# refresh-bio/colord

Measured on AMD Instinct MI355X. Metric: input Gbases/s + archive size vs ref, ONT 50 Gb at 1/2/4/8 MI355X, higher is better.
Workload: dtype u64

## Files before the change

### colord_amd/csrc/anchors.hip

```cpp
#include "common.hpp"
#include "objects.hpp"
#include <algorithm>

struct cl_anchors {
	cl_ctx* ctx = nullptr;
	uint32_t n_reads = 0, c = 0;
	uint64_t n_anchors = 0;
	DevBuf<uint32_t> n_cands;
	DevBuf<uint32_t> cand;
	DevBuf<uint64_t> cand_off;
	DevBuf<uint32_t> anchors;
};

namespace {

struct Arena { const uint64_t* packed; const uint64_t* word_off; const uint32_t* lens; };

__device__ inline uint64_t mmer_at(const Arena& A, uint64_t wb, uint32_t p, uint32_t m)
{
	const uint64_t* w = A.packed + wb + (p >> 5);
	const uint32_t j = p & 31;
	const uint64_t hi = w[0], lo = w[1];
	const uint32_t s = 128 - 2 * (j + m);
	const uint64_t v = (s >= 64) ? (hi >> (s - 64)) : ((hi << (64 - s)) | (lo >> s));
	return v & ((1ULL << (2 * m)) - 1);
}
__device__ inline uint64_t mmer_of(uint64_t hi, uint64_t lo, uint32_t p, uint32_t m)
{
	const uint32_t s = 128 - 2 * ((p & 31) + m);
	const uint64_t v = (s >= 64) ? (hi >> (s - 64)) : ((hi << (64 - s)) | (lo >> s));
	return v & ((1ULL << (2 * m)) - 1);
}
__device__ inline uint64_t revcomp_m(uint64_t x, uint32_t m)
{
	x = ~x; x = __brevll(x);
	x = ((x >> 1) & 0x5555555555555555ULL) | ((x & 0x5555555555555555ULL) << 1);
	return x >> (64 - 2 * m);
}
__device__ inline uint64_t ref_mmer(const Arena& R, uint32_t id, bool rev, uint32_t q, uint32_t m)
{
	const uint32_t len = R.lens[id];
	const uint64_t wb = R.word_off[id];
	return rev ? revcomp_m(mmer_at(R, wb, len - m - q, m), m) : mmer_at(R, wb, q, m);
}

struct BuildSlot { uint64_t key; uint32_t head; uint32_t strands; };
typedef uint2 EncSlot;
constexpr uint32_t LINK_POS = 0x3fffffffu;
__device__ inline uint32_t tag_of(uint64_t hash) { return (uint32_t)((hash * 0xD6E8FEB86659FD93ULL) >> 32); }
__device__ inline uint32_t table_slot(uint64_t hash, uint32_t tsz) { return (uint32_t)(((uint64_t)(uint32_t)(hash >> 17) * tsz) >> 32); }
struct EncTable { EncSlot* slots; const uint64_t* toff; uint32_t* next; const uint64_t* noff; };
constexpr uint32_t REGION_SLOTS = 2048;
constexpr uint64_t KEY_EMPTY = ~0ULL;
constexpr uint32_t NIL = 0xffffffffu;

__global__ void k_table_sizes(const uint32_t* __restrict__ lens, const uint8_t* __restrict__ has_n, const uint32_t* __restrict__ ncand,
                              uint32_t r0, uint32_t r1, uint32_t m, uint32_t x4, uint32_t lds_max_n, uint32_t* __restrict__ tsize, uint32_t* __restrict__ nsize, uint32_t* __restrict__ err)
{
	uint32_t r = r0 + blockIdx.x * blockDim.x + threadIdx.x;
	if (r >= r1) return;
	uint32_t len = lens[r];
	bool active = ncand[r] > 0 && !has_n[r] && len >= m;
	uint32_t n = active ? len - m + 1 : 0;
	if (n <= lds_max_n) n = 0;
	uint32_t t = 0;
	if (n) { t = 16; while (t < 2 * n + n / 2 && t < REGION_SLOTS) t <<= 1; if (t >= REGION_SLOTS) t = (uint32_t)(((uint64_t)n * x4 / 4 + REGION_SLOTS - 1) / REGION_SLOTS * REGION_SLOTS); }
	tsize[r - r0] = t; nsize[r - r0] = n;
}
constexpr uint32_t REGION = REGION_SLOTS, INS_T = 256;
__global__ __launch_bounds__(INS_T) void k_table_insert(Arena A, uint32_t r0, uint32_t r1, uint32_t m, EncTable T, uint32_t* __restrict__ n_distinct,
                                                       uint2* __restrict__ bins , uint32_t* __restrict__ err)
{
	__shared__ BuildSlot reg[REGION];
	__shared__ uint32_t cnt[512], start[513];
	const uint32_t r = r0 + blockIdx.x;
	if (r >= r1) return;
	const uint64_t t0 = T.toff[r - r0]; const uint32_t tsz = (uint32_t)(T.toff[r - r0 + 1] - t0);
	if (!tsz) return;
	const uint64_t n0 = T.noff[r - r0]; const uint32_t n = (uint32_t)(T.noff[r - r0 + 1] - n0);
	const uint64_t wb = A.word_off[r];
	const uint32_t lane = threadIdx.x & 63;
	const uint32_t rs = tsz < REGION ? tsz : REGION, n_reg = tsz / rs, rshift = 31 - (uint32_t)__clz((int)rs);
	uint2* bin = bins + n0;
	uint32_t fresh = 0;
	for (uint32_t rg0 = 0; rg0 < n_reg; rg0 += 512)
	{
		const uint32_t nr = n_reg - rg0 < 512 ? n_reg - rg0 : 512;
		for (uint32_t i = threadIdx.x; i < 512; i += INS_T) cnt[i] = 0;
		__syncthreads();
		for (uint32_t p = threadIdx.x; p < n; p += INS_T)
		{
			const uint64_t xf = mmer_at(A, wb, p, m), xr = revcomp_m(xf, m), x = xf < xr ? xf : xr;
			const uint32_t h = table_slot(hash_mm(x), tsz), rg = (h >> rshift) - rg0;
			if (rg < nr) atomicAdd(&cnt[rg], 1u);
		}
		__syncthreads();
		if (threadIdx.x == 0) { uint32_t a = 0; for (uint32_t i = 0; i < nr; ++i) { start[i] = a; a += cnt[i]; cnt[i] = 0; } start[nr] = a; }
		__syncthreads();
		for (uint32_t p = threadIdx.x; p < n; p += INS_T)
		{
			const uint64_t xf = mmer_at(A, wb, p, m), xr = revcomp_m(xf, m), x = xf < xr ? xf : xr;
			const uint32_t h = table_slot(hash_mm(x), tsz), rg = (h >> rshift) - rg0;
			if (rg < nr) bin[start[rg] + atomicAdd(&cnt[rg], 1u)] = make_uint2(p, h);
		}
		__syncthreads();
		__threadfence_block();
		for (uint32_t rg = 0; rg < nr; ++rg)
		{
			for (uint32_t i = threadIdx.x; i < rs; i += INS_T) { reg[i].key = KEY_EMPTY; reg[i].head = NIL; reg[i].strands = 0; }
			__syncthreads();
			const uint32_t b = start[rg], e = start[rg + 1];
			for (uint32_t i = b + threadIdx.x; i < e; i += INS_T)
			{
				const uint2 ph = bin[i];
				const uint32_t pp = ph.x;
				const uint64_t xf = mmer_at(A, wb, pp, m), xr = revcomp_m(xf, m), x = xf < xr ? xf : xr;
				uint32_t off = ph.y & (rs - 1), tries = 0;
				for (;;)
				{
					unsigned long long old = atomicCAS((unsigned long long*)&reg[off].key, (unsigned long long)KEY_EMPTY, (unsigned long long)x);
					if (old == KEY_EMPTY || old == x) break;
					off = (off + 1) & (rs - 1);
					if (++tries > rs) { atomicOr(err, 2u); break; }
				}
				const uint32_t strand = xf != x ? 1u : 0u;
				T.next[n0 + pp] = atomicExch(&reg[off].head, pp | (strand << 31));
				if (!(atomicOr(&reg[off].strands, 1u << strand) & (1u << strand))) ++fresh;
			}
			__syncthreads();
			EncSlot* dst = T.slots + t0 + (uint64_t)(rg0 + rg) * rs;
			for (uint32_t i = threadIdx.x; i < rs; i += INS_T) dst[i] = make_uint2(reg[i].head == NIL ? 0u : tag_of(hash_mm(reg[i].key)), reg[i].head);
			__syncthreads();
		}
	}
	fresh = wave_sum(fresh);
	if (lane == 0 && fresh) atomicAdd(&n_distinct[r - r0], fresh);
}
struct TaskCfg { uint32_t r0, r1, c, m; uint32_t pe, pr; double frac_always, frac_min, max_mult; };

constexpr uint32_t FILT_WORDS = 2048, STAGE = 128;
__device__ inline uint32_t filt_word(uint64_t hash) { return (uint32_t)(hash >> 46) & (FILT_WORDS - 1); }
__device__ inline uint64_t filt_mask(uint64_t hash) { return (1ull << ((hash >> 40) & 63)) | (1ull << ((hash >> 34) & 63)) | (1ull << ((hash >> 28) & 63)); }
__device__ __host__ inline uint32_t match_segments(uint32_t n, uint32_t seg_n) { return (seg_n == 0 || n <= seg_n + seg_n / 2) ? 1u : (n + seg_n - 1) / seg_n; }
__global__ __launch_bounds__(256) void k_match(Arena A, Arena R, EncTable T, TaskCfg cfg, const uint32_t* __restrict__ cand_refs, const uint32_t* __restrict__ cand_n,
                                              const uint32_t* __restrict__ n_distinct, const uint2* __restrict__ work , uint32_t n_work, uint32_t seg_n,
                                              unsigned long long* __restrict__ n_pairs, uint64_t cap, uint64_t* __restrict__ pairs)
{
	__shared__ unsigned long long filt[FILT_WORDS];
	__shared__ uint64_t stage_all[4][STAGE];
	if (blockIdx.x >= n_work) return;
	const uint32_t rl = work[blockIdx.x].x, seg = work[blockIdx.x].y;
	const uint32_t lane = threadIdx.x & 63, wv = threadIdx.x >> 6;
	const uint32_t r = cfg.r0 + rl;
	const uint64_t t0 = T.toff[rl]; const uint32_t tsz = (uint32_t)(T.toff[rl + 1] - t0);
	const uint32_t n_slots = cand_n[r] < cfg.c ? cand_n[r] : cfg.c;
	if (tsz == 0 || n_slots == 0) return;
	const uint32_t elen = A.lens[r];
	if ((double)n_distinct[rl] < cfg.frac_min * (double)elen && !((double)n_distinct[rl] > cfg.frac_always * (double)elen)) return;
	for (uint32_t i = threadIdx.x; i < FILT_WORDS; i += 256) filt[i] = 0;
	__syncthreads();
	uint32_t p_lo, p_hi;
	{
		const uint64_t ewb = A.word_off[r]; const uint32_t n = elen - cfg.m + 1;
		const uint32_t nseg = match_segments(n, seg_n);
		if (seg >= nseg) return;
		p_lo = (uint32_t)((uint64_t)n * seg / nseg); p_hi = (uint32_t)((uint64_t)n * (seg + 1) / nseg);
		for (uint32_t p = p_lo + threadIdx.x; p < p_hi; p += 256)
		{
			const uint64_t xf = mmer_at(A, ewb, p, cfg.m), xr = revcomp_m(xf, cfg.m);
			const uint64_t hash = hash_mm(xf < xr ? xf : xr);
			atomicOr(&filt[filt_word(hash)], (unsigned long long)filt_mask(hash));
		}
	}
	__syncthreads();
	const uint64_t n0 = T.noff[rl];
	const uint64_t ewb = A.word_off[r];
	uint64_t* stage = stage_all[wv]; uint32_t fill = 0;
	auto flush = [&]() {
		if (!fill) return;
		unsigned long long base = 0;
		if (lane == 0) base = atomicAdd(n_pairs, (unsigned long long)fill);
		base = ((unsigned long long)__shfl((int)(base >> 32), 0, 64) << 32) | (uint32_t)__shfl((int)(uint32_t)base, 0, 64);
		if (base + fill <= cap) for (uint32_t i = lane; i < fill; i += 64) pairs[base + i] = stage[i];
		fill = 0;
	};
	for (uint32_t slot = 0; slot < n_slots; ++slot)
	{
		const uint32_t id = cand_refs[(uint64_t)r * cfg.c + slot], rlen = R.lens[id];
		if (rlen < cfg.m) continue;
		const uint64_t rwb = R.word_off[id];
		const uint32_t nq = rlen - cfg.m + 1, sl = rl * cfg.c + slot;
		const uint32_t PR = cfg.pr; const uint32_t pr_mask = (1u << PR) - 1;
		const uint64_t key_rev = (uint64_t)(2 * sl) << (cfg.pe + PR), key_fwd = (uint64_t)(2 * sl + 1) << (cfg.pe + PR);
		if (threadIdx.x == 0 && seg == 0) atomicAdd(n_pairs + 1, (unsigned long long)nq);
		const uint64_t* rw = R.packed + rwb;
		struct Probe { uint64_t x; uint2 slot; uint32_t h, tag; bool pass, fwd_other, rev_other; };
		auto probe = [&](uint32_t q, uint64_t hi, uint64_t lo) -> Probe
		{
			Probe P{ 0, make_uint2(0u, NIL), 0, 0, false, false, false };
			if (q < nq)
			{
				const uint64_t y = mmer_of(hi, lo, q, cfg.m), z = revcomp_m(y, cfg.m), x = y < z ? y : z;
				const uint64_t hash = hash_mm(x);
				const uint64_t fm = filt_mask(hash);
				if ((filt[filt_word(hash)] & fm) == fm)
				{
					P.pass = true; P.x = x; P.fwd_other = y != x; P.rev_other = z != x;
					P.h = table_slot(hash, tsz); P.tag = tag_of(hash);
					P.slot = T.slots[t0 + P.h];
				}
			}
			return P;
		};
		uint64_t hi1 = 0, lo1 = 0, hi2 = 0, lo2 = 0;
		Probe cur;
		{
			const uint32_t q = wv * 64 + lane;
			uint64_t hi = 0, lo = 0;
			if (q < nq) { hi = rw[q >> 5]; lo = rw[(q >> 5) + 1]; }
			if (q + 256 < nq) { hi1 = rw[(q + 256) >> 5]; lo1 = rw[((q + 256) >> 5) + 1]; }
			cur = probe(q, hi, lo);
		}
		const uint32_t rmask = (tsz < REGION ? tsz : REGION) - 1;
		for (uint32_t q0 = wv * 64; q0 < nq; q0 += 256)
		{
			const uint32_t q = q0 + lane;
			hi2 = 0; lo2 = 0;
			if (q + 512 < nq) { hi2 = rw[(q + 512) >> 5]; lo2 = rw[((q + 512) >> 5) + 1]; }
			const Probe nxt = probe(q + 256, hi1, lo1);
			uint32_t head = NIL, cnt = 0;
			const uint32_t fs = cur.fwd_other ? 1u : 0u, rs_ = cur.rev_other ? 1u : 0u;
			if (cur.pass)
			{
				uint2 sl8 = cur.slot; uint32_t h = cur.h;
				while (sl8.y != NIL)
				{
					if (sl8.x == cur.tag)
					{
						const uint64_t xf = mmer_at(A, ewb, sl8.y & LINK_POS, cfg.m), xr = revcomp_m(xf, cfg.m);
						if ((xf < xr ? xf : xr) == cur.x) { head = sl8.y; break; }
					}
					h = (h & ~rmask) | ((h + 1) & rmask);
					sl8 = T.slots[t0 + h];
				}
				for (uint32_t p = head; p != NIL; p = T.next[n0 + (p & LINK_POS)])
					if ((p & LINK_POS) >= p_lo && (p & LINK_POS) < p_hi) cnt += (uint32_t)((p >> 31) == fs) + (uint32_t)((p >> 31) == rs_);
			}
			cur = nxt; hi1 = hi2; lo1 = lo2;
			if (!__any(cnt != 0)) continue;
			const uint32_t incl = wave_incl_scan(cnt), tot = __shfl(incl, 63, 64);
			const uint64_t kf = key_fwd | (uint64_t)(~q & pr_mask), kr = key_rev | (uint64_t)(~(nq - 1 - q) & pr_mask);
			if (fill + tot > STAGE) flush();
			if (tot <= STAGE)
			{
				uint32_t o = fill + incl - cnt;
				for (uint32_t p = head; p != NIL; p = T.next[n0 + (p & LINK_POS)])
				{
					if ((p & LINK_POS) < p_lo || (p & LINK_POS) >= p_hi) continue;
					const uint64_t pos = (uint64_t)(p & LINK_POS) << PR;
					if ((p >> 31) == fs) stage[o++] = kf | pos;
					if ((p >> 31) == rs_) stage[o++] = kr | pos;
				}
				fill += tot;
				continue;
			}
			unsigned long long base = 0;
			if (lane == 0) base = atomicAdd(n_pairs, (unsigned long long)tot);
			base = ((unsigned long long)__shfl((int)(base >> 32), 0, 64) << 32) | (uint32_t)__shfl((int)(uint32_t)base, 0, 64);
			if (base + tot > cap) continue;
			uint64_t o = base + incl - cnt;
			for (uint32_t p = head; p != NIL; p = T.next[n0 + (p & LINK_POS)])
			{
				if ((p & LINK_POS) < p_lo || (p & LINK_POS) >= p_hi) continue;
				const uint64_t pos = (uint64_t)(p & LINK_POS) << PR;
				if ((p >> 31) == fs) pairs[o++] = kf | pos;
				if ((p >> 31) == rs_) pairs[o++] = kr | pos;
			}
		}
	}
	flush();
}
template<uint32_t MAXN> struct LdsGeom { static constexpr uint32_t SLOTS = ((MAXN + MAXN / 2) + 17) & ~1u, WORDS = (MAXN + 27 + 31) / 32 + 2; };
__device__ inline uint32_t lds_table_slots(uint32_t n) { const uint32_t s = (n + n / 2 + 1) & ~1u; return s < 16 ? 16 : s; }
template<uint32_t MAXN, uint32_t FW, uint32_t NT, uint32_t WAVES_PER_SIMD>
__global__ __launch_bounds__(NT, WAVES_PER_SIMD) void k_match_lds(Arena A, Arena R, TaskCfg cfg, uint32_t min_n, const uint8_t* __restrict__ has_n,
                                                 const uint32_t* __restrict__ cand_refs, const uint32_t* __restrict__ cand_n, uint32_t* __restrict__ n_distinct, uint32_t n_reads,
                                                 unsigned long long* __restrict__ n_pairs, uint64_t cap, uint64_t* __restrict__ pairs, uint32_t dbg)
{
	static_assert(MAXN <= 65535 && (FW & (FW - 1)) == 0 && NT % 64 == 0, "positions are 16-bit links; 0xffff is the empty slot");
	constexpr uint32_t NW = NT / 64, LSTAGE = 64;
	__shared__ unsigned long long filt[FW];
	__shared__ uint64_t rd[LdsGeom<MAXN>::WORDS];
	__shared__ uint32_t slots32[LdsGeom<MAXN>::SLOTS / 2];
	__shared__ uint64_t stage_all[NW][LSTAGE];
	__shared__ uint32_t s_distinct;
	const uint32_t rl = blockIdx.x;
	if (rl >= n_reads) return;
	const uint32_t r = cfg.r0 + rl, m = cfg.m;
	const uint32_t elen = A.lens[r];
	const uint32_t n_slots = cand_n[r] < cfg.c ? cand_n[r] : cfg.c;
	if (n_slots == 0 || has_n[r] || elen < m) return;
	const uint32_t n = elen - m + 1;
	if (n <= min_n || n > MAXN) return;
	const uint32_t lane = threadIdx.x & 63, wv = threadIdx.x >> 6;
	const uint32_t S = lds_table_slots(n);
	const uint16_t* slot16 = (const uint16_t*)slots32;
	{
		const uint64_t* src = A.packed + A.word_off[r];
		const uint32_t nw = (elen + 31) / 32 + 1;
		for (uint32_t i = threadIdx.x; i < nw; i += NT) rd[i] = src[i];
		for (uint32_t i = threadIdx.x; i < FW; i += NT) filt[i] = 0;
		for (uint32_t i = threadIdx.x; i < S / 2; i += NT) slots32[i] = 0xffffffffu;
		if (threadIdx.x == 0) s_distinct = 0;
	}
	__syncthreads();
	if (dbg == 1) return;
	auto own = [&](uint32_t p) -> uint64_t { return mmer_of(rd[p >> 5], rd[(p >> 5) + 1], p, m); };
	auto step = [&](uint32_t off) -> uint32_t { return off + 1 == S ? 0u : off + 1; };
	{
		uint32_t fresh = 0;
		for (uint32_t p = threadIdx.x; p < n; p += NT)
		{
			const uint64_t xf = own(p), xr = revcomp_m(xf, m), hash = hash_mm(xf < xr ? xf : xr);
			atomicOr(&filt[(uint32_t)(hash >> 46) & (FW - 1)], (unsigned long long)filt_mask(hash));
			bool dup = false;
			for (uint32_t off = table_slot(hash, S);;)
			{
				uint32_t* w = &slots32[off >> 1]; const uint32_t sh = (off & 1) * 16;
				const uint32_t old = *(volatile uint32_t*)w, q = (old >> sh) & 0xffffu;
				if (q != 0xffffu) { if (!dup && own(q) == xf) dup = true; off = step(off); continue; }
				if (atomicCAS(w, old, (old & ~(0xffffu << sh)) | (p << sh)) == old) break;
			}
			fresh += dup ? 0u : 1u;
		}
		fresh = wave_sum(fresh);
		if (lane == 0 && fresh) atomicAdd(&s_distinct, fresh);
	}
	__syncthreads();
	const uint32_t nd = s_distinct;
	if (threadIdx.x == 0) n_distinct[rl] = nd;
	if (dbg == 2) return;
	if ((double)nd < cfg.frac_min * (double)elen && !((double)nd > cfg.frac_always * (double)elen)) return;
	uint64_t* stage = stage_all[wv]; uint32_t fill = 0;
	auto flush = [&]() {
		if (!fill) return;
		unsigned long long base = 0;
		if (lane == 0) base = atomicAdd(n_pairs, (unsigned long long)fill);
		base = ((unsigned long long)__shfl((int)(base >> 32), 0, 64) << 32) | (uint32_t)__shfl((int)(uint32_t)base, 0, 64);
		if (base + fill <= cap) for (uint32_t i = lane; i < fill; i += 64) pairs[base + i] = stage[i];
		fill = 0;
	};
	struct Look { uint64_t y, z; uint32_t h0, cnt, nh, hp0, hp1, hf0, hf1; };
	auto look = [&](bool live, uint32_t q, uint64_t hi, uint64_t lo) -> Look {
		Look L{ 0, 0, 0, 0, 0, 0, 0, 0, 0 };
		if (!live) return L;
		L.y = mmer_of(hi, lo, q, m); L.z = revcomp_m(L.y, m);
		const uint64_t hash = hash_mm(L.y < L.z ? L.y : L.z), fm = filt_mask(hash);
		if ((filt[(uint32_t)(hash >> 46) & (FW - 1)] & fm) != fm || dbg == 3) return L;
		L.h0 = table_slot(hash, S);
		for (uint32_t off = L.h0;; off = step(off))
// ... 366 lines not shown
		const uint64_t s = (uint64_t)r * c + i;
		if (i < n)
		{
			const uint32_t t = sel_task[i] & 0x7fffffffu, slot = (t / 2) % c;
			o_cand[4 * s] = cand_refs[(uint64_t)r * c + slot]; o_cand[4 * s + 1] = (t & 1) == 0 ? 1u : 0u;
			o_cand[4 * s + 2] = sel_tot[i]; o_cand[4 * s + 3] = sel_n[i];
			o_task[(uint64_t)rl * c + i] = sel_task[i]; o_count[(uint64_t)rl * c + i] = sel_n[i];
		}
		else { o_cand[4 * s] = ~0u; o_cand[4 * s + 1] = 0; o_cand[4 * s + 2] = 0; o_cand[4 * s + 3] = 0; o_task[(uint64_t)rl * c + i] = ~0u; o_count[(uint64_t)rl * c + i] = 0; }
	}
}
__global__ void k_copy_fix(const uint32_t* __restrict__ o_task, const uint64_t* __restrict__ slot_off, uint64_t n_slots,
                           const uint64_t* __restrict__ pair_off, const uint32_t* __restrict__ anch, uint64_t dst_base, uint32_t* __restrict__ out,
                           TaskCfg cfg, const uint32_t* __restrict__ kanch, const uint64_t* __restrict__ common_off, uint64_t common_base)
{
	const uint64_t s = (uint64_t)blockIdx.x * blockDim.x + threadIdx.x;
	if (s >= n_slots) return;
	const uint32_t tm = o_task[s];
	if (tm == ~0u) return;
	const uint32_t t = tm & 0x7fffffffu;
	const uint32_t n = (uint32_t)(slot_off[s + 1] - slot_off[s]);
	const uint32_t* src = anch + 3 * pair_off[t];
	if (tm & 0x80000000u)
	{
		const uint64_t gs = (uint64_t)cfg.r0 * cfg.c + t / 2;
		const uint64_t o = common_off[gs] - common_base; const uint32_t nk = (uint32_t)(common_off[gs + 1] - common_off[gs]);
		src = kanch + 6 * o + (uint64_t)(t & 1) * 3 * nk;
	}
	uint32_t* dst = out + 3 * (dst_base + slot_off[s]);
	for (uint32_t i = 0; i < 3 * n; ++i) dst[i] = src[i];
	for (uint32_t i = 0; i + 1 < n; ++i)
	{
		const uint32_t end = dst[3 * i + 2] + dst[3 * i];
		if (dst[3 * (i + 1) + 2] < end) { const uint32_t d = end - dst[3 * (i + 1) + 2]; dst[3 * (i + 1) + 2] += d; dst[3 * (i + 1)] -= d; dst[3 * (i + 1) + 1] += d; }
	}
	for (uint32_t i = 0; i + 1 < n; ++i)
	{
		const uint32_t end = dst[3 * i + 1] + dst[3 * i];
		if (dst[3 * (i + 1) + 1] < end) { const uint32_t d = end - dst[3 * (i + 1) + 1]; dst[3 * (i + 1) + 1] += d; dst[3 * (i + 1)] -= d; dst[3 * (i + 1) + 2] += d; }
	}
}
__global__ void k_add_u64(uint64_t* v, uint64_t n, uint64_t c) { uint64_t i = (uint64_t)blockIdx.x * blockDim.x + threadIdx.x; if (i < n) v[i] += c; }
}

extern "C" cl_status cl_anchor_candidates_hifi(cl_ctx* ctx, const cl_reads* reads, const cl_reads* refs, const uint32_t* d_cand_refs, const uint32_t* d_cand_n,
                                               uint32_t c, uint32_t anchor_len, double frac_always, double frac_min, double max_matches_mult,
                                               uint32_t min_anchors, uint32_t kmer_len, uint32_t modulo, const uint64_t* d_common_off, const uint64_t* d_common, cl_anchors** out);
extern "C" cl_status cl_anchor_candidates(cl_ctx* ctx, const cl_reads* reads, const cl_reads* refs, const uint32_t* d_cand_refs, const uint32_t* d_cand_n,
                                          uint32_t c, uint32_t anchor_len, double frac_always, double frac_min, double max_matches_mult,
                                          uint32_t min_anchors, cl_anchors** out)
{
	return cl_anchor_candidates_hifi(ctx, reads, refs, d_cand_refs, d_cand_n, c, anchor_len, frac_always, frac_min, max_matches_mult, min_anchors, 0, 0, nullptr, nullptr, out);
}
extern "C" cl_status cl_anchor_candidates_hifi(cl_ctx* ctx, const cl_reads* reads, const cl_reads* refs, const uint32_t* d_cand_refs, const uint32_t* d_cand_n,
                                               uint32_t c, uint32_t anchor_len, double frac_always, double frac_min, double max_matches_mult,
                                               uint32_t min_anchors, uint32_t kmer_len, uint32_t modulo, const uint64_t* d_common_off, const uint64_t* d_common, cl_anchors** out)
{
	if (!ctx || !reads || !refs || !d_cand_refs || !d_cand_n || !out) return cl_fail(ctx, CL_E_INVALID, "cl_anchor_candidates: null argument");
	const bool hifi = d_common_off != nullptr;
	if (hifi && (kmer_len < 2 || kmer_len > 28 || modulo == 0)) return cl_fail(ctx, CL_E_INVALID, "cl_anchor_candidates_hifi: 2 <= kmer_len <= 28, modulo >= 1");
	if (c == 0 || c > 16 || anchor_len < 2 || anchor_len > 28) return cl_fail(ctx, CL_E_INVALID, "cl_anchor_candidates: 1 <= c <= 16, 2 <= anchor_len <= 28");
	HIP_TRY(ctx, hipSetDevice(ctx->device));
	const uint32_t nr = reads->n_reads, m = anchor_len;
	cl_anchors* X = new cl_anchors(); X->ctx = ctx; X->n_reads = nr; X->c = c;
	std::unique_ptr<cl_anchors> guard(X);
	DEV_ALLOC(ctx, X->n_cands, nr); DEV_ALLOC(ctx, X->cand, (uint64_t)nr * c * 4); DEV_ALLOC(ctx, X->cand_off, (uint64_t)nr * c + 1);
	Arena A{ reads->packed.p, reads->word_off.p, reads->lens.p }, R{ refs->packed.p, refs->word_off.p, refs->lens.p };
	std::vector<uint32_t> h_len(nr);
	if (nr) HIP_TRY(ctx, hipMemcpy(h_len.data(), reads->lens.p, (uint64_t)nr * 4, hipMemcpyDeviceToHost));
	auto bits_for = [](uint64_t v) -> uint32_t { uint32_t b = 1; while ((1ull << b) <= v) ++b; return b; };
	uint32_t max_ref_len = 0;
	if (refs->n_reads)
	{
		std::vector<uint32_t> rl(refs->n_reads);
		HIP_TRY(ctx, hipMemcpy(rl.data(), refs->lens.p, (uint64_t)refs->n_reads * 4, hipMemcpyDeviceToHost));
		for (uint32_t l : rl) max_ref_len = std::max(max_ref_len, l);
	}
	const uint32_t pr_bits = bits_for(max_ref_len);
	const uint64_t BATCH_BASES = 1ull << 28;
	std::vector<DevBuf<uint32_t>> chunks; std::vector<uint64_t> chunk_n;
	uint64_t total_anchors = 0;
	double pairs_per_base = 0.5;
	struct TableBatch {
		uint32_t r0 = 0, r1 = 0, pe = 1; uint64_t acc = 0, nsum = 0;
		DevBuf<uint32_t> n_distinct, next, err; DevBuf<uint64_t> toff, noff; DevBuf<EncSlot> slots; DevBuf<uint2> bins;
		std::vector<uint2> h_work; DevBuf<uint2> work;
		struct SideSync { hipStream_t s = nullptr; ~SideSync() { if (s) (void)hipStreamSynchronize(s); } } sync;
	};
	HIP_TRY(ctx, cl_side_stream(ctx, ctx->side));
	constexpr uint32_t LDS_N_A = 12288, LDS_N_B = 24576, LDS_NT = 1024;
	uint32_t lds_max_n = 0;
	if (const char* e = getenv("COLORD_HIP_ANCHORS_LDS")) lds_max_n = atoi(e) <= 0 ? 0u : (uint32_t)atoi(e) <= LDS_N_A ? LDS_N_A : LDS_N_B;
	const uint32_t match_seg = getenv("COLORD_HIP_MATCH_SEG") ? (uint32_t)std::max(0, atoi(getenv("COLORD_HIP_MATCH_SEG"))) : 16384u;
	const uint32_t lds_dbg = getenv("COLORD_HIP_LDS_DBG") ? (uint32_t)atoi(getenv("COLORD_HIP_LDS_DBG")) : 0u;
	auto prepare = [&](uint32_t r0, std::unique_ptr<TableBatch>& out) -> cl_status {
		out = std::make_unique<TableBatch>();
		TableBatch& B = *out;
		uint32_t r1 = r0; uint64_t acc = 0;
		uint32_t mx = 0;
		while (r1 < nr && (r1 == r0 || acc + h_len[r1] <= BATCH_BASES))
		{
			const uint32_t pe = bits_for(std::max(mx, h_len[r1]));
			if (r1 > r0 && pe + pr_bits + bits_for((r1 - r0 + 1) * 2 * c) > 64) break;
			mx = std::max(mx, h_len[r1]); acc += h_len[r1]; ++r1;
		}
		B.r0 = r0; B.r1 = r1; B.acc = acc; B.pe = bits_for(mx);
		for (uint32_t r = r0; r < r1; ++r)
			for (uint32_t sg = 0, ns = match_segments(h_len[r] >= m ? h_len[r] - m + 1 : 0, match_seg); sg < ns; ++sg) B.h_work.push_back(make_uint2(r - r0, sg));
		if (B.pe + pr_bits + bits_for((r1 - r0) * 2 * c) > 64) return cl_fail(ctx, CL_E_UNSUPPORTED, "cl_anchor_candidates: a read and its candidates are too long for 64-bit match keys");
		const uint32_t nb = r1 - r0;
		const uint32_t table_x4 = 8;
		LaunchOn on(ctx, ctx->side);
		B.sync.s = ctx->side;
		DevBuf<uint32_t> tsize, nsize, err; DEV_ALLOC(ctx, tsize, nb); DEV_ALLOC(ctx, nsize, nb); DEV_ALLOC(ctx, err, 1); DEV_ALLOC(ctx, B.n_distinct, nb);
		HIP_TRY(ctx, hipMemsetAsync(err.p, 0, 4, ctx->side));
		LAUNCH(ctx, k_table_sizes, grid_for(nb, 256), 256, (const uint32_t*)reads->lens.p, (const uint8_t*)reads->has_n.p, d_cand_n, r0, r1, m, table_x4, lds_max_n, tsize.p, nsize.p, err.p);
		DEV_ALLOC(ctx, B.toff, (uint64_t)nb + 1); DEV_ALLOC(ctx, B.noff, (uint64_t)nb + 1);
		uint64_t tsum = 0;
		CL_TRY(dev_exclusive_scan_u64(ctx, tsize.p, B.toff.p, nb, &tsum));
		CL_TRY(dev_exclusive_scan_u64(ctx, nsize.p, B.noff.p, nb, &B.nsum));
		uint32_t herr = 0; HIP_TRY(ctx, hipMemcpyAsync(&herr, err.p, 4, hipMemcpyDeviceToHost, ctx->side)); HIP_TRY(ctx, hipStreamSynchronize(ctx->side));
		DEV_ALLOC(ctx, B.slots, tsum); DEV_ALLOC(ctx, B.next, B.nsum); DEV_ALLOC(ctx, B.bins, B.nsum); DEV_ALLOC(ctx, B.err, 1);
		DEV_ALLOC(ctx, B.work, B.h_work.size() + 1);
		if (!B.h_work.empty()) HIP_TRY(ctx, hipMemcpyAsync(B.work.p, B.h_work.data(), B.h_work.size() * sizeof(uint2), hipMemcpyHostToDevice, ctx->side));
		HIP_TRY(ctx, hipMemsetAsync(B.n_distinct.p, 0, (uint64_t)nb * 4, ctx->side));
		HIP_TRY(ctx, hipMemsetAsync(B.err.p, 0, 4, ctx->side));
		EncTable T{ B.slots.p, B.toff.p, B.next.p, B.noff.p };
		LAUNCHB(ctx, B.nsum * (0.25 + 16.0) , k_table_insert, nb, INS_T, A, r0, r1, m, T, B.n_distinct.p, B.bins.p, B.err.p);
		HIP_TRY(ctx, hipGetLastError());
		return CL_OK;
	};
	std::unique_ptr<TableBatch> cur, nxt;
	if (nr) CL_TRY(prepare(0, cur));
	while (cur)
	{
		const uint32_t r0 = cur->r0, r1 = cur->r1; const uint64_t acc = cur->acc;
		const uint32_t nb = r1 - r0, n_tasks = nb * 2 * c;
		TaskCfg cfg{ r0, r1, c, m, cur->pe, pr_bits, frac_always, frac_min, max_matches_mult };
		HIP_TRY(ctx, hipStreamSynchronize(ctx->stream));
		HIP_TRY(ctx, hipStreamSynchronize(ctx->side));
		cur->sync.s = nullptr;
		{ uint32_t herr = 0; HIP_TRY(ctx, hipMemcpy(&herr, cur->err.p, 4, hipMemcpyDeviceToHost)); if (herr) return cl_fail(ctx, CL_E_UNSUPPORTED, "cl_anchor_candidates: a region of an m-mer table overflowed"); }
		DevBuf<uint32_t>& n_distinct = cur->n_distinct;
		EncTable T{ cur->slots.p, cur->toff.p, cur->next.p, cur->noff.p };
		DevBuf<uint32_t> pair_cnt; DEV_ALLOC(ctx, pair_cnt, (uint64_t)n_tasks + 1);
		DevBuf<uint64_t> pair_off; DEV_ALLOC(ctx, pair_off, (uint64_t)n_tasks + 1);
		DevBuf<unsigned long long> d_np; DEV_ALLOC(ctx, d_np, 4);
		DevBuf<uint64_t> pairs;
		uint64_t n_pairs = 0;
		for (uint64_t cap = (uint64_t)(pairs_per_base * 1.25 * (double)acc) + (1u << 20);;)
		{
			DEV_ALLOC(ctx, pairs, cap);
			HIP_TRY(ctx, hipMemsetAsync(d_np.p, 0, 32, ctx->stream));
			if (lds_max_n)
			{
				LAUNCH_NAMED(ctx, "k_match_lds<12288>", (k_match_lds<LDS_N_A, 2048, LDS_NT, 8>), nb, LDS_NT, A, R, cfg, 0u, (const uint8_t*)reads->has_n.p, d_cand_refs, d_cand_n, n_distinct.p, nb, d_np.p, cap, pairs.p, lds_dbg);
				if (lds_max_n > LDS_N_A)
					LAUNCH_NAMED(ctx, "k_match_lds<24576>", (k_match_lds<LDS_N_B, 4096, LDS_NT, 4>), nb, LDS_NT, A, R, cfg, LDS_N_A, (const uint8_t*)reads->has_n.p, d_cand_refs, d_cand_n, n_distinct.p, nb, d_np.p, cap, pairs.p, lds_dbg);
			}
			LAUNCHB(ctx, 0.0, k_match, (uint32_t)cur->h_work.size(), 256, A, R, T, cfg, d_cand_refs, d_cand_n, (const uint32_t*)n_distinct.p, (const uint2*)cur->work.p, (uint32_t)cur->h_work.size(), match_seg, d_np.p, cap, pairs.p);
			HIP_TRY(ctx, hipGetLastError());
			unsigned long long h_np2[2] = { 0, 0 };
			HIP_TRY(ctx, hipMemcpyAsync(h_np2, d_np.p, 16, hipMemcpyDeviceToHost, ctx->stream));
			if (r1 < nr && !nxt) CL_TRY(prepare(r1, nxt));
			HIP_TRY(ctx, hipStreamSynchronize(ctx->stream));
			const unsigned long long h_np = h_np2[0];
			n_pairs = h_np;
			if (ctx->timing && !ctx->pending_bytes.empty()) ctx->pending_bytes.back() = (double)h_np2[1] * 8.25 + (double)std::min<uint64_t>(h_np, cap) * 8.0;
			if (getenv("COLORD_HIP_ANCHOR_DEBUG")) fprintf(stderr, "[anchors] batch reads %u..%u bases %llu: pairs %llu cap %llu\n", r0, r1, (unsigned long long)acc, h_np, (unsigned long long)cap);
			if (n_pairs >= (1ull << 32)) return cl_fail(ctx, CL_E_UNSUPPORTED, "cl_anchor_candidates: batch produces >= 2^32 match pairs");
			if (n_pairs <= cap) break;
			cap = n_pairs;
		}
		if (acc) pairs_per_base = std::max(pairs_per_base, (double)n_pairs / (double)acc);
		DevBuf<int> tf, ts, pred; DEV_ALLOC(ctx, tf, n_pairs); DEV_ALLOC(ctx, ts, n_pairs); DEV_ALLOC(ctx, pred, n_pairs);
		DevBuf<uint32_t> anch; DEV_ALLOC(ctx, anch, 3 * n_pairs);
		DevBuf<uint32_t> t_nanch, t_tot; DEV_ALLOC(ctx, t_nanch, n_tasks); DEV_ALLOC(ctx, t_tot, n_tasks);
		if (n_pairs)
		{
			uint32_t tb = 1; while ((1ull << tb) < n_tasks) ++tb;
			CL_TRY(dev_sort_pairs(ctx, pairs.p, nullptr, n_pairs, 0, cfg.pe + cfg.pr + tb));
		}
		LAUNCH(ctx, k_task_pairs, grid_for((uint64_t)n_tasks + 1, 256), 256, (const uint64_t*)pairs.p, n_pairs, A, cfg, (const uint32_t*)n_distinct.p, n_tasks, pair_off.p, pair_cnt.p);
		LAUNCHB(ctx, n_pairs * 32.0, k_lis_anchors, grid_for(n_tasks, 64), 64, A, R, cfg, d_cand_refs, n_tasks, (const uint64_t*)pair_off.p, (const uint32_t*)pair_cnt.p, (const uint64_t*)pairs.p,
			tf.p, ts.p, pred.p, anch.p, t_nanch.p, t_tot.p, (uint32_t)(getenv("COLORD_HIP_LIS_DBG") ? atoi(getenv("COLORD_HIP_LIS_DBG")) : 0));
		HIP_TRY(ctx, hipGetLastError());
		const uint64_t n_slots = (uint64_t)nb * c;
		DevBuf<uint64_t> k_sorted; DevBuf<uint32_t> k_tab, kanch, k_n, k_tot; DevBuf<uint8_t> k_use;
		uint64_t common_base = 0;
		if (hifi)
		{
			uint64_t hb[2] = { 0, 0 };
			HIP_TRY(ctx, hipMemcpy(&hb[0], d_common_off + (uint64_t)r0 * c, 8, hipMemcpyDeviceToHost));
			HIP_TRY(ctx, hipMemcpy(&hb[1], d_common_off + (uint64_t)r1 * c, 8, hipMemcpyDeviceToHost));
			common_base = hb[0];
			const uint64_t nk = hb[1] - hb[0];
			DEV_ALLOC(ctx, k_sorted, nk + 1); DEV_ALLOC(ctx, k_tab, 8 * nk + 8); DEV_ALLOC(ctx, kanch, 6 * nk + 6);
			DEV_ALLOC(ctx, k_n, 2 * n_slots); DEV_ALLOC(ctx, k_tot, 2 * n_slots); DEV_ALLOC(ctx, k_use, n_slots);
			KmerArgs ka{ d_common, d_common_off, k_sorted.p, k_tab.p, kanch.p, k_n.p, k_tot.p, k_use.p, common_base, kmer_len, make_modtest(modulo) };
			LAUNCH(ctx, k_kmer_anchors, grid_for(n_slots, 64), 64, A, R, cfg, d_cand_refs, d_cand_n, (const uint8_t*)reads->has_n.p, (const uint32_t*)n_distinct.p, ka);
			HIP_TRY(ctx, hipGetLastError());
		}
		DevBuf<uint32_t> o_task, o_count; DEV_ALLOC(ctx, o_task, n_slots); DEV_ALLOC(ctx, o_count, n_slots);
		LAUNCH(ctx, k_select, grid_for(nb, 128), 128, cfg, d_cand_refs, d_cand_n, min_anchors, (const uint32_t*)t_nanch.p, (const uint32_t*)t_tot.p,
			(const uint8_t*)(hifi ? k_use.p : nullptr), (const uint32_t*)k_n.p, (const uint32_t*)k_tot.p,
			X->n_cands.p, X->cand.p, o_task.p, o_count.p);
		DevBuf<uint64_t> slot_off; DEV_ALLOC(ctx, slot_off, n_slots + 1);
		uint64_t n_here = 0;
		CL_TRY(dev_exclusive_scan_u64(ctx, o_count.p, slot_off.p, n_slots, &n_here));
		DevBuf<uint32_t> chunk; DEV_ALLOC(ctx, chunk, 3 * n_here);
		LAUNCH(ctx, k_copy_fix, grid_for(n_slots, 128), 128, (const uint32_t*)o_task.p, (const uint64_t*)slot_off.p, n_slots, (const uint64_t*)pair_off.p,
			(const uint32_t*)anch.p, (uint64_t)0, chunk.p, cfg, (const uint32_t*)kanch.p, d_common_off, common_base);
		HIP_TRY(ctx, hipMemcpyAsync(X->cand_off.p + (uint64_t)r0 * c, slot_off.p, n_slots * 8, hipMemcpyDeviceToDevice, ctx->stream));
		if (total_anchors) LAUNCH(ctx, k_add_u64, grid_for(n_slots, 256), 256, X->cand_off.p + (uint64_t)r0 * c, n_slots, total_anchors);
		HIP_TRY(ctx, hipGetLastError());
		HIP_TRY(ctx, hipStreamSynchronize(ctx->stream));
		chunks.push_back(std::move(chunk)); chunk_n.push_back(n_here);
		total_anchors += n_here;
		cur = std::move(nxt);
	}
	X->n_anchors = total_anchors;
	DEV_ALLOC(ctx, X->anchors, 3 * total_anchors);
	uint64_t o = 0;
	for (size_t i = 0; i < chunks.size(); ++i)
	{
		if (chunk_n[i]) HIP_TRY(ctx, hipMemcpyAsync(X->anchors.p + 3 * o, chunks[i].p, chunk_n[i] * 12, hipMemcpyDeviceToDevice, ctx->stream));
		o += chunk_n[i];
	}
	HIP_TRY(ctx, hipMemcpyAsync(X->cand_off.p + (uint64_t)nr * c, &total_anchors, 8, hipMemcpyHostToDevice, ctx->stream));
	HIP_TRY(ctx, hipStreamSynchronize(ctx->stream));
	cl_timing_collect(ctx);
	*out = guard.release();
	return CL_OK;
}
extern "C" void cl_anchors_free(cl_anchors* a) { delete a; }
extern "C" uint64_t cl_anchors_total(const cl_anchors* a) { return a->n_anchors; }
extern "C" const uint32_t* cl_anchors_n_cands(const cl_anchors* a) { return a->n_cands.p; }
extern "C" const uint32_t* cl_anchors_cands(const cl_anchors* a) { return a->cand.p; }
extern "C" const uint64_t* cl_anchors_cand_offsets(const cl_anchors* a) { return a->cand_off.p; }
extern "C" const uint32_t* cl_anchors_data(const cl_anchors* a) { return a->anchors.p; }
```

Measured before the change: 3.003.

## Store chain links in binned records and tile-stage the region binning

Removes the separate `next` array. Each binned record (position, next link) now serves as the chain node, so match-time chain walks read one contiguous uint2 per hop instead of indexing `next` by position and the table build writes one array. Binning scatter is reworked to rank entries per 2048-element tile in shared memory, scan offsets, then write to the global bins in region order, which aims for coalesced writes. Small tables (one region) skip binning entirely and insert directly. It also adds an error-path stream sync and extra debug output, at the cost of more complex indexing, since slot heads now refer to bin indices rather than read positions.

```diff
diff --git a/colord_amd/csrc/anchors.hip b/colord_amd/csrc/anchors.hip
--- a/colord_amd/csrc/anchors.hip
+++ b/colord_amd/csrc/anchors.hip
@@ -49,7 +49,7 @@
 constexpr uint32_t LINK_POS = 0x3fffffffu;
 __device__ inline uint32_t tag_of(uint64_t hash) { return (uint32_t)((hash * 0xD6E8FEB86659FD93ULL) >> 32); }
 __device__ inline uint32_t table_slot(uint64_t hash, uint32_t tsz) { return (uint32_t)(((uint64_t)(uint32_t)(hash >> 17) * tsz) >> 32); }
-struct EncTable { EncSlot* slots; const uint64_t* toff; uint32_t* next; const uint64_t* noff; };
+struct EncTable { EncSlot* slots; const uint64_t* toff; uint2* bins ; const uint64_t* noff; };
 constexpr uint32_t REGION_SLOTS = 2048;
 constexpr uint64_t KEY_EMPTY = ~0ULL;
 constexpr uint32_t NIL = 0xffffffffu;
@@ -67,26 +67,62 @@
 	if (n) { t = 16; while (t < 2 * n + n / 2 && t < REGION_SLOTS) t <<= 1; if (t >= REGION_SLOTS) t = (uint32_t)(((uint64_t)n * x4 / 4 + REGION_SLOTS - 1) / REGION_SLOTS * REGION_SLOTS); }
 	tsize[r - r0] = t; nsize[r - r0] = n;
 }
-constexpr uint32_t REGION = REGION_SLOTS, INS_T = 256;
-__global__ __launch_bounds__(INS_T) void k_table_insert(Arena A, uint32_t r0, uint32_t r1, uint32_t m, EncTable T, uint32_t* __restrict__ n_distinct,
-                                                       uint2* __restrict__ bins , uint32_t* __restrict__ err)
+constexpr uint32_t REGION = REGION_SLOTS, INS_T = 256, BIN_TILE = 2048, BIN_PER = BIN_TILE / INS_T;
+static_assert(BIN_TILE * sizeof(uint2) + (512 + INS_T / 64) * sizeof(uint32_t) <= REGION * sizeof(BuildSlot), "the binning tile and its offsets alias reg[]");
+__global__ __launch_bounds__(INS_T) void k_table_insert(Arena A, uint32_t r0, uint32_t r1, uint32_t m, EncTable T, uint32_t* __restrict__ n_distinct, uint32_t* __restrict__ err)
 {
 	__shared__ BuildSlot reg[REGION];
-	__shared__ uint32_t cnt[512], start[513];
+	__shared__ uint32_t cnt[512], start[513], tcnt[512];
 	const uint32_t r = r0 + blockIdx.x;
 	if (r >= r1) return;
 	const uint64_t t0 = T.toff[r - r0]; const uint32_t tsz = (uint32_t)(T.toff[r - r0 + 1] - t0);
 	if (!tsz) return;
 	const uint64_t n0 = T.noff[r - r0]; const uint32_t n = (uint32_t)(T.noff[r - r0 + 1] - n0);
 	const uint64_t wb = A.word_off[r];
-	const uint32_t lane = threadIdx.x & 63;
+	const uint32_t lane = threadIdx.x & 63, wv = threadIdx.x >> 6;
 	const uint32_t rs = tsz < REGION ? tsz : REGION, n_reg = tsz / rs, rshift = 31 - (uint32_t)__clz((int)rs);
-	uint2* bin = bins + n0;
+	uint2* bin = T.bins + n0;
+	uint2* stage = reinterpret_cast<uint2*>(reg);
+	uint32_t* toff = reinterpret_cast<uint32_t*>(stage + BIN_TILE);
+	uint32_t* wtot = toff + 512;
 	uint32_t fresh = 0;
-	for (uint32_t rg0 = 0; rg0 < n_reg; rg0 += 512)
+	auto insert = [&](uint32_t i, uint32_t pp, uint32_t h)
+	{
+		const uint64_t xf = mmer_at(A, wb, pp, m), xr = revcomp_m(xf, m), x = xf < xr ? xf : xr;
+		uint32_t off = h & (rs - 1), tries = 0;
+		for (;;)
+		{
+			unsigned long long old = atomicCAS((unsigned long long*)&reg[off].key, (unsigned long long)KEY_EMPTY, (unsigned long long)x);
+			if (old == KEY_EMPTY || old == x) break;
+			off = (off + 1) & (rs - 1);
+			if (++tries > rs) { atomicOr(err, 2u); break; }
+		}
+		const uint32_t strand = xf != x ? 1u : 0u;
+		bin[i] = make_uint2(pp, atomicExch(&reg[off].head, i | (strand << 31)));
+		if (!(atomicOr(&reg[off].strands, 1u << strand) & (1u << strand))) ++fresh;
+	};
+	auto clear_region = [&]() { for (uint32_t i = threadIdx.x; i < rs; i += INS_T) { reg[i].key = KEY_EMPTY; reg[i].head = NIL; reg[i].strands = 0; } };
+	auto store_region = [&](uint32_t rg)
+	{
+		EncSlot* dst = T.slots + t0 + (uint64_t)rg * rs;
+		for (uint32_t i = threadIdx.x; i < rs; i += INS_T) dst[i] = make_uint2(reg[i].head == NIL ? 0u : tag_of(hash_mm(reg[i].key)), reg[i].head);
+	};
+	if (n_reg == 1)
+	{
+		clear_region();
+		__syncthreads();
+		for (uint32_t p = threadIdx.x; p < n; p += INS_T)
+		{
+			const uint64_t xf = mmer_at(A, wb, p, m), xr = revcomp_m(xf, m);
+			insert(p, p, table_slot(hash_mm(xf < xr ? xf : xr), tsz));
+		}
+		__syncthreads();
+		store_region(0);
+	}
+	else for (uint32_t rg0 = 0, base = 0; rg0 < n_reg; rg0 += 512)
 	{
 		const uint32_t nr = n_reg - rg0 < 512 ? n_reg - rg0 : 512;
-		for (uint32_t i = threadIdx.x; i < 512; i += INS_T) cnt[i] = 0;
+		for (uint32_t i = threadIdx.x; i < 512; i += INS_T) { cnt[i] = 0; tcnt[i] = 0; }
 		__syncthreads();
 		for (uint32_t p = threadIdx.x; p < n; p += INS_T)
 		{
@@ -95,43 +131,63 @@
 			if (rg < nr) atomicAdd(&cnt[rg], 1u);
 		}
 		__syncthreads();
-		if (threadIdx.x == 0) { uint32_t a = 0; for (uint32_t i = 0; i < nr; ++i) { start[i] = a; a += cnt[i]; cnt[i] = 0; } start[nr] = a; }
+		if (threadIdx.x == 0) { uint32_t a = base; for (uint32_t i = 0; i < nr; ++i) { start[i] = a; a += cnt[i]; cnt[i] = start[i]; } start[nr] = a; }
 		__syncthreads();
-		for (uint32_t p = threadIdx.x; p < n; p += INS_T)
-		{
-			const uint64_t xf = mmer_at(A, wb, p, m), xr = revcomp_m(xf, m), x = xf < xr ? xf : xr;
-			const uint32_t h = table_slot(hash_mm(x), tsz), rg = (h >> rshift) - rg0;
-			if (rg < nr) bin[start[rg] + atomicAdd(&cnt[rg], 1u)] = make_uint2(p, h);
-		}
-		__syncthreads();
+		for (uint32_t p0 = 0; p0 < n; p0 += BIN_TILE)
+		{
+			uint32_t hh[BIN_PER], rk[BIN_PER];
+#pragma unroll
+			for (uint32_t j = 0; j < BIN_PER; ++j)
+			{
+				const uint32_t p = p0 + j * INS_T + threadIdx.x;
+				hh[j] = 0; rk[j] = NIL;
+				if (p < n)
+				{
+					const uint64_t xf = mmer_at(A, wb, p, m), xr = revcomp_m(xf, m), x = xf < xr ? xf : xr;
+					hh[j] = table_slot(hash_mm(x), tsz);
+					const uint32_t rg = (hh[j] >> rshift) - rg0;
+					if (rg < nr) rk[j] = atomicAdd(&tcnt[rg], 1u);
+				}
+			}
+			__syncthreads();
+			{
+				const uint32_t a = tcnt[2 * threadIdx.x], b = tcnt[2 * threadIdx.x + 1], incl = wave_incl_scan(a + b);
+				if (lane == 63) wtot[wv] = incl;
+				__syncthreads();
+				uint32_t ex = incl - (a + b);
+				for (uint32_t w = 0; w < wv; ++w) ex += wtot[w];
+				toff[2 * threadIdx.x] = ex; toff[2 * threadIdx.x + 1] = ex + a;
+			}
+			__syncthreads();
+			uint32_t tile_n = 0;
+			for (uint32_t w = 0; w < INS_T / 64; ++w) tile_n += wtot[w];
+#pragma unroll
+			for (uint32_t j = 0; j < BIN_PER; ++j)
+				if (rk[j] != NIL) stage[toff[(hh[j] >> rshift) - rg0] + rk[j]] = make_uint2(p0 + j * INS_T + threadIdx.x, hh[j]);
+			__syncthreads();
+			for (uint32_t i = threadIdx.x; i < tile_n; i += INS_T)
+			{
+				const uint2 e = stage[i];
+				const uint32_t rg = (e.y >> rshift) - rg0;
+				bin[cnt[rg] + (i - toff[rg])] = e;
+			}
+			__syncthreads();
+			for (uint32_t i = threadIdx.x; i < 512; i += INS_T) { cnt[i] += tcnt[i]; tcnt[i] = 0; }
+			__syncthreads();
+		}
 		__threadfence_block();
 		for (uint32_t rg = 0; rg < nr; ++rg)
 		{
-			for (uint32_t i = threadIdx.x; i < rs; i += INS_T) { reg[i].key = KEY_EMPTY; reg[i].head = NIL; reg[i].strands = 0; }
+			clear_region();
 			__syncthreads();
 			const uint32_t b = start[rg], e = start[rg + 1];
-			for (uint32_t i = b + threadIdx.x; i < e; i += INS_T)
-			{
-				const uint2 ph = bin[i];
-				const uint32_t pp = ph.x;
-				const uint64_t xf = mmer_at(A, wb, pp, m), xr = revcomp_m(xf, m), x = xf < xr ? xf : xr;
-				uint32_t off = ph.y & (rs - 1), tries = 0;
-				for (;;)
-				{
-					unsigned long long old = atomicCAS((unsigned long long*)&reg[off].key, (unsigned long long)KEY_EMPTY, (unsigned long long)x);
-					if (old == KEY_EMPTY || old == x) break;
-					off = (off + 1) & (rs - 1);
-					if (++tries > rs) { atomicOr(err, 2u); break; }
-				}
-				const uint32_t strand = xf != x ? 1u : 0u;
-				T.next[n0 + pp] = atomicExch(&reg[off].head, pp | (strand << 31));
-				if (!(atomicOr(&reg[off].strands, 1u << strand) & (1u << strand))) ++fresh;
-			}
+			for (uint32_t i = b + threadIdx.x; i < e; i += INS_T) { const uint2 ph = bin[i]; insert(i, ph.x, ph.y); }
 			__syncthreads();
-			EncSlot* dst = T.slots + t0 + (uint64_t)(rg0 + rg) * rs;
-			for (uint32_t i = threadIdx.x; i < rs; i += INS_T) dst[i] = make_uint2(reg[i].head == NIL ? 0u : tag_of(hash_mm(reg[i].key)), reg[i].head);
+			store_region(rg0 + rg);
 			__syncthreads();
 		}
+		base = start[nr];
+		__syncthreads();
 	}
 	fresh = wave_sum(fresh);
 	if (lane == 0 && fresh) atomicAdd(&n_distinct[r - r0], fresh);
@@ -175,6 +231,15 @@
 	__syncthreads();
 	const uint64_t n0 = T.noff[rl];
 	const uint64_t ewb = A.word_off[r];
+	auto walk = [&](uint32_t l, uint2 rec, auto&& f)
+	{
+		while (l != NIL)
+		{
+			f(rec.x, l >> 31);
+			l = rec.y;
+			if (l != NIL) rec = T.bins[n0 + (l & LINK_POS)];
+		}
+	};
 	uint64_t* stage = stage_all[wv]; uint32_t fill = 0;
 	auto flush = [&]() {
 		if (!fill) return;
@@ -229,6 +294,7 @@
 			if (q + 512 < nq) { hi2 = rw[(q + 512) >> 5]; lo2 = rw[((q + 512) >> 5) + 1]; }
 			const Probe nxt = probe(q + 256, hi1, lo1);
 			uint32_t head = NIL, cnt = 0;
+			uint2 hrec = make_uint2(0u, NIL);
 			const uint32_t fs = cur.fwd_other ? 1u : 0u, rs_ = cur.rev_other ? 1u : 0u;
 			if (cur.pass)
 			{
@@ -237,14 +303,14 @@
 				{
 					if (sl8.x == cur.tag)
 					{
-						const uint64_t xf = mmer_at(A, ewb, sl8.y & LINK_POS, cfg.m), xr = revcomp_m(xf, cfg.m);
-						if ((xf < xr ? xf : xr) == cur.x) { head = sl8.y; break; }
+						const uint2 rec = T.bins[n0 + (sl8.y & LINK_POS)];
+						const uint64_t xf = mmer_at(A, ewb, rec.x, cfg.m), xr = revcomp_m(xf, cfg.m);
+						if ((xf < xr ? xf : xr) == cur.x) { head = sl8.y; hrec = rec; break; }
 					}
 					h = (h & ~rmask) | ((h + 1) & rmask);
 					sl8 = T.slots[t0 + h];
 				}
-				for (uint32_t p = head; p != NIL; p = T.next[n0 + (p & LINK_POS)])
-					if ((p & LINK_POS) >= p_lo && (p & LINK_POS) < p_hi) cnt += (uint32_t)((p >> 31) == fs) + (uint32_t)((p >> 31) == rs_);
+				walk(head, hrec, [&](uint32_t pos, uint32_t strand) { if (pos >= p_lo && pos < p_hi) cnt += (uint32_t)(strand == fs) + (uint32_t)(strand == rs_); });
 			}
 			cur = nxt; hi1 = hi2; lo1 = lo2;
 			if (!__any(cnt != 0)) continue;
@@ -254,13 +320,13 @@
 			if (tot <= STAGE)
 			{
 				uint32_t o = fill + incl - cnt;
-				for (uint32_t p = head; p != NIL; p = T.next[n0 + (p & LINK_POS)])
+				walk(head, hrec, [&](uint32_t p, uint32_t strand)
 				{
-					if ((p & LINK_POS) < p_lo || (p & LINK_POS) >= p_hi) continue;
-					const uint64_t pos = (uint64_t)(p & LINK_POS) << PR;
-					if ((p >> 31) == fs) stage[o++] = kf | pos;
-					if ((p >> 31) == rs_) stage[o++] = kr | pos;
-				}
+					if (p < p_lo || p >= p_hi) return;
+					const uint64_t pos = (uint64_t)p << PR;
+					if (strand == fs) stage[o++] = kf | pos;
+					if (strand == rs_) stage[o++] = kr | pos;
+				});
 				fill += tot;
 				continue;
 			}
@@ -269,13 +335,13 @@
 			base = ((unsigned long long)__shfl((int)(base >> 32), 0, 64) << 32) | (uint32_t)__shfl((int)(uint32_t)base, 0, 64);
 			if (base + tot > cap) continue;
 			uint64_t o = base + incl - cnt;
-			for (uint32_t p = head; p != NIL; p = T.next[n0 + (p & LINK_POS)])
-			{
-				if ((p & LINK_POS) < p_lo || (p & LINK_POS) >= p_hi) continue;
-				const uint64_t pos = (uint64_t)(p & LINK_POS) << PR;
-				if ((p >> 31) == fs) pairs[o++] = kf | pos;
-				if ((p >> 31) == rs_) pairs[o++] = kr | pos;
-			}
+			walk(head, hrec, [&](uint32_t p, uint32_t strand)
+			{
+				if (p < p_lo || p >= p_hi) return;
+				const uint64_t pos = (uint64_t)p << PR;
+				if (strand == fs) pairs[o++] = kf | pos;
+				if (strand == rs_) pairs[o++] = kr | pos;
+			});
 		}
 	}
 	flush();
@@ -808,8 +874,8 @@
 	uint64_t total_anchors = 0;
 	double pairs_per_base = 0.5;
 	struct TableBatch {
-		uint32_t r0 = 0, r1 = 0, pe = 1; uint64_t acc = 0, nsum = 0;
-		DevBuf<uint32_t> n_distinct, next, err; DevBuf<uint64_t> toff, noff; DevBuf<EncSlot> slots; DevBuf<uint2> bins;
+		uint32_t r0 = 0, r1 = 0, pe = 1; uint64_t acc = 0, nsum = 0, tsum = 0;
+		DevBuf<uint32_t> n_distinct, err; DevBuf<uint64_t> toff, noff; DevBuf<EncSlot> slots; DevBuf<uint2> bins;
 		std::vector<uint2> h_work; DevBuf<uint2> work;
 		struct SideSync { hipStream_t s = nullptr; ~SideSync() { if (s) (void)hipStreamSynchronize(s); } } sync;
 	};
@@ -842,17 +908,17 @@
 		HIP_TRY(ctx, hipMemsetAsync(err.p, 0, 4, ctx->side));
 		LAUNCH(ctx, k_table_sizes, grid_for(nb, 256), 256, (const uint32_t*)reads->lens.p, (const uint8_t*)reads->has_n.p, d_cand_n, r0, r1, m, table_x4, lds_max_n, tsize.p, nsize.p, err.p);
 		DEV_ALLOC(ctx, B.toff, (uint64_t)nb + 1); DEV_ALLOC(ctx, B.noff, (uint64_t)nb + 1);
-		uint64_t tsum = 0;
+		uint64_t& tsum = B.tsum;
 		CL_TRY(dev_exclusive_scan_u64(ctx, tsize.p, B.toff.p, nb, &tsum));
 		CL_TRY(dev_exclusive_scan_u64(ctx, nsize.p, B.noff.p, nb, &B.nsum));
 		uint32_t herr = 0; HIP_TRY(ctx, hipMemcpyAsync(&herr, err.p, 4, hipMemcpyDeviceToHost, ctx->side)); HIP_TRY(ctx, hipStreamSynchronize(ctx->side));
-		DEV_ALLOC(ctx, B.slots, tsum); DEV_ALLOC(ctx, B.next, B.nsum); DEV_ALLOC(ctx, B.bins, B.nsum); DEV_ALLOC(ctx, B.err, 1);
+		DEV_ALLOC(ctx, B.slots, tsum); DEV_ALLOC(ctx, B.bins, B.nsum); DEV_ALLOC(ctx, B.err, 1);
 		DEV_ALLOC(ctx, B.work, B.h_work.size() + 1);
 		if (!B.h_work.empty()) HIP_TRY(ctx, hipMemcpyAsync(B.work.p, B.h_work.data(), B.h_work.size() * sizeof(uint2), hipMemcpyHostToDevice, ctx->side));
 		HIP_TRY(ctx, hipMemsetAsync(B.n_distinct.p, 0, (uint64_t)nb * 4, ctx->side));
 		HIP_TRY(ctx, hipMemsetAsync(B.err.p, 0, 4, ctx->side));
-		EncTable T{ B.slots.p, B.toff.p, B.next.p, B.noff.p };
-		LAUNCHB(ctx, B.nsum * (0.25 + 16.0) , k_table_insert, nb, INS_T, A, r0, r1, m, T, B.n_distinct.p, B.bins.p, B.err.p);
+		EncTable T{ B.slots.p, B.toff.p, B.bins.p, B.noff.p };
+		LAUNCHB(ctx, B.nsum * (0.25 + 16.0) , k_table_insert, nb, INS_T, A, r0, r1, m, T, B.n_distinct.p, B.err.p);
 		HIP_TRY(ctx, hipGetLastError());
 		return CL_OK;
 	};
@@ -868,7 +934,7 @@
 		cur->sync.s = nullptr;
 		{ uint32_t herr = 0; HIP_TRY(ctx, hipMemcpy(&herr, cur->err.p, 4, hipMemcpyDeviceToHost)); if (herr) return cl_fail(ctx, CL_E_UNSUPPORTED, "cl_anchor_candidates: a region of an m-mer table overflowed"); }
 		DevBuf<uint32_t>& n_distinct = cur->n_distinct;
-		EncTable T{ cur->slots.p, cur->toff.p, cur->next.p, cur->noff.p };
+		EncTable T{ cur->slots.p, cur->toff.p, cur->bins.p, cur->noff.p };
 		DevBuf<uint32_t> pair_cnt; DEV_ALLOC(ctx, pair_cnt, (uint64_t)n_tasks + 1);
 		DevBuf<uint64_t> pair_off; DEV_ALLOC(ctx, pair_off, (uint64_t)n_tasks + 1);
 		DevBuf<unsigned long long> d_np; DEV_ALLOC(ctx, d_np, 4);
@@ -888,12 +954,16 @@
 			HIP_TRY(ctx, hipGetLastError());
 			unsigned long long h_np2[2] = { 0, 0 };
 			HIP_TRY(ctx, hipMemcpyAsync(h_np2, d_np.p, 16, hipMemcpyDeviceToHost, ctx->stream));
-			if (r1 < nr && !nxt) CL_TRY(prepare(r1, nxt));
+			if (r1 < nr && !nxt)
+			{
+				const cl_status st = prepare(r1, nxt);
+				if (st != CL_OK) { (void)hipStreamSynchronize(ctx->stream); return st; }
+			}
 			HIP_TRY(ctx, hipStreamSynchronize(ctx->stream));
 			const unsigned long long h_np = h_np2[0];
 			n_pairs = h_np;
 			if (ctx->timing && !ctx->pending_bytes.empty()) ctx->pending_bytes.back() = (double)h_np2[1] * 8.25 + (double)std::min<uint64_t>(h_np, cap) * 8.0;
-			if (getenv("COLORD_HIP_ANCHOR_DEBUG")) fprintf(stderr, "[anchors] batch reads %u..%u bases %llu: pairs %llu cap %llu\n", r0, r1, (unsigned long long)acc, h_np, (unsigned long long)cap);
+			if (getenv("COLORD_HIP_ANCHOR_DEBUG")) fprintf(stderr, "[anchors] batch reads %u..%u bases %llu: table slots %llu records %llu pairs %llu cap %llu\n", r0, r1, (unsigned long long)acc, (unsigned long long)cur->tsum, (unsigned long long)cur->nsum, h_np, (unsigned long long)cap);
 			if (n_pairs >= (1ull << 32)) return cl_fail(ctx, CL_E_UNSUPPORTED, "cl_anchor_candidates: batch produces >= 2^32 match pairs");
 			if (n_pairs <= cap) break;
 			cap = n_pairs;
```

Result: no change. 2.977 (-0.9%).
